# jinbeizame007/pytorch-r2d2-DPG

Hardware: NVIDIA H100
Metric: learner sequence-steps/sec (batch x seq_len) (higher is better)
Workload: dtype bf16x3 (fp32 operands split into bf16 hi+lo, three tensor-core passes, fp32 accumulate: ~16-bit operands)

## Files before the change

### pytorch-r2d2-dpg_b200/csrc/lstm_scan.cu

```cuda
#include <cooperative_groups.h>
#include <stdlib.h>

#include "gemm.cuh"
#include "lstm_scan.cuh"
#include "elementwise.cuh"
#include "sm90.cuh"

namespace cg = cooperative_groups;

namespace r2d2 {
namespace {

constexpr int SCAN_THREADS = 256;
constexpr int UNITS_PER_CTA = 32;
constexpr int ROWS_PER_CTA = 128;
constexpr int GT_LD = ROWS_PER_CTA + 4;
constexpr int DG_LD = ROWS_PER_CTA + 8;
constexpr unsigned long long kWaitLimitNs = 4000000000ull;

__device__ unsigned g_scan_status = 0;

__device__ __forceinline__ float accurate_sigmoid(float x) { return 1.0f / (1.0f + expf(-x)); }

__device__ __forceinline__ unsigned long long global_ns() {
  unsigned long long t;
  asm volatile("mov.u64 %0, %globaltimer;" : "=l"(t));
  return t;
}

__device__ __forceinline__ void wait_slice(uint64_t* bar, uint32_t parity) {
  if (sm90::mbar_try_wait(bar, parity)) return;
  if (*reinterpret_cast<volatile unsigned*>(&g_scan_status)) return;
  const unsigned long long t0 = global_ns();
  while (!sm90::mbar_try_wait(bar, parity)) {
    if (global_ns() - t0 > kWaitLimitNs) {
      atomicExch(&g_scan_status, 1u);
      return;
    }
  }
}

__device__ __forceinline__ uint32_t slice_parity(int s) { return (uint32_t)((s - 1) >> 1) & 1u; }

template <int H> __host__ __device__ constexpr bool w_hi_in_smem() { return H > 256; }

template <int H, int NB>
struct FwdSmem {
  static constexpr int C = H / 32;
  static constexpr int HROW = UNITS_PER_CTA + 8;
  static constexpr int SLICE = 2 * NB * HROW;
  static constexpr int W_BYTES = w_hi_in_smem<H>() ? (H / 16) * 8 * 32 * 16 : 0;
  static constexpr int HB_ELEMS = 2 * C * SLICE;
  static constexpr int GT_ELEMS = NB * GT_LD;
  static constexpr int HS_ELEMS = SLICE;
  static constexpr int BAR_OFF = W_BYTES + HB_ELEMS * 2 + GT_ELEMS * 4 + HS_ELEMS * 2;
  static constexpr int BYTES = BAR_OFF + 2 * C * 8;
  static_assert((SLICE * 2) % 16 == 0 && BAR_OFF % 16 == 0, "bulk copies need 16-byte granules");
  static_assert(BYTES <= 232448, "forward scan tile does not fit in 227 KB of shared memory");
};

template <int H, int NB>
__global__ void __launch_bounds__(SCAN_THREADS, 1) lstm_scan_fwd_kernel(ScanFwdParams p) {
  constexpr int C = H / 32, KS = H / 16, NT = NB / 8;
  constexpr bool WS = w_hi_in_smem<H>();
  using SM = FwdSmem<H, NB>;
  constexpr int HROW = SM::HROW, SLICE = SM::SLICE;
  cg::cluster_group cluster = cg::this_cluster();
  const int rank = (int)cluster.block_rank();
  const int b0 = (blockIdx.x / C) * NB;
  const int tid = threadIdx.x, lane = tid & 31, w = tid >> 5;
  const int g = lane >> 2, c = lane & 3;
  const int B = p.B, S = p.T * p.repeat;

  extern __shared__ __align__(16) unsigned char smem_raw[];
  uint4* w_hi_s = reinterpret_cast<uint4*>(smem_raw);
  __nv_bfloat16* hb = reinterpret_cast<__nv_bfloat16*>(smem_raw + SM::W_BYTES);
  float* gt = reinterpret_cast<float*>(smem_raw + SM::W_BYTES + SM::HB_ELEMS * 2);
  __nv_bfloat16* hstage = reinterpret_cast<__nv_bfloat16*>(smem_raw + SM::W_BYTES + SM::HB_ELEMS * 2 + SM::GT_ELEMS * 4);
  uint64_t* bar = reinterpret_cast<uint64_t*>(smem_raw + SM::BAR_OFF);

  for (int idx = tid; idx < NB * H; idx += SCAN_THREADS) {
    const int n = idx / H, k = idx % H, b = b0 + n;
    float v = (b < B && p.h0) ? __ldg(p.h0 + (size_t)b * H + k) : 0.f;
    __nv_bfloat16 hi, lo;
    split_bf16(v, hi, lo);
    __nv_bfloat16* row = hb + (0 * C + k / UNITS_PER_CTA) * SLICE + n * HROW + k % UNITS_PER_CTA;
    row[0] = hi;
    row[NB * HROW] = lo;
  }
  const int ug = rank * 32 + lane;
  float cst[NT];
#pragma unroll
  for (int e = 0; e < NT; ++e) {
    const int b = b0 + w + 8 * e;
    cst[e] = 0.f;
    if (b < B) {
      float hv = p.h0 ? __ldg(p.h0 + (size_t)b * H + ug) : 0.f;
      float cv = p.c0 ? __ldg(p.c0 + (size_t)b * H + ug) : 0.f;
      p.hs[(size_t)b * H + ug] = hv;
      p.cs[(size_t)b * H + ug] = cv;
      cst[e] = cv;
    }
  }
  if (tid < 2 * C) {
    sm90::mbar_init(bar + tid, 1);
    sm90::fence_mbar_init_cluster();
    sm90::mbar_arrive_expect_tx(bar + tid, SLICE * 2);
  }

  uint32_t a_hi[WS ? 1 : KS][4], a_lo[KS][4];
  {
    const int gate = w >> 1;
    const int u_lo = (w & 1) * 16 + g;
    const float* w_r0 = p.whh + (size_t)(gate * H + rank * 32 + u_lo) * H;
    const float* w_r1 = w_r0 + (size_t)8 * H;
#pragma unroll
    for (int ks = 0; ks < KS; ++ks) {
      const int k = ks * 16 + 2 * c;
      float2 v0 = __ldg(reinterpret_cast<const float2*>(w_r0 + k));
      float2 v1 = __ldg(reinterpret_cast<const float2*>(w_r1 + k));
      float2 v2 = __ldg(reinterpret_cast<const float2*>(w_r0 + k + 8));
      float2 v3 = __ldg(reinterpret_cast<const float2*>(w_r1 + k + 8));
      uint32_t h[4];
      split_pack2(v0.x, v0.y, h[0], a_lo[ks][0]);
      split_pack2(v1.x, v1.y, h[1], a_lo[ks][1]);
      split_pack2(v2.x, v2.y, h[2], a_lo[ks][2]);
      split_pack2(v3.x, v3.y, h[3], a_lo[ks][3]);
      if constexpr (WS) {
        w_hi_s[(ks * 8 + w) * 32 + lane] = make_uint4(h[0], h[1], h[2], h[3]);
      } else {
#pragma unroll
        for (int f = 0; f < 4; ++f) a_hi[ks][f] = h[f];
      }
    }
  }
  __syncthreads();
  cluster.sync();

  const size_t gstride = (size_t)4 * H;
  for (int s = 0; s < S; ++s) {
    const int cur = s & 1, nxt = cur ^ 1;
    const int t = s / p.repeat;

#pragma unroll
    for (int nt = 0; nt < NT; ++nt)
#pragma unroll
      for (int f = 0; f < 4; ++f) {
        const int n = nt * 8 + 2 * c + (f & 1), r = 16 * w + g + (f >> 1) * 8, b = b0 + n;
        if (b < B) sm90::cp_async_4(gt + n * GT_LD + r, p.gin + ((size_t)t * B + b) * gstride + (r >> 5) * H + rank * 32 + (r & 31));
      }
    sm90::cp_async_commit();

    float acc[NT][4];
#pragma unroll
    for (int nt = 0; nt < NT; ++nt)
#pragma unroll
      for (int e = 0; e < 4; ++e) acc[nt][e] = 0.f;
    const __nv_bfloat16* hb_cur = hb + cur * C * SLICE;
    uint64_t* bar_cur = bar + cur * C;
    const uint32_t parity = slice_parity(s);
#pragma unroll
    for (int ks = 0; ks < KS; ++ks) {
      if ((ks & 1) == 0 && s > 0) wait_slice(bar_cur + ks / 2, parity);
      const __nv_bfloat16* hb_hi = hb_cur + (ks / 2) * SLICE;
      const __nv_bfloat16* hb_lo = hb_hi + NB * HROW;
      uint32_t ah[4];
      if constexpr (WS) {
        const uint4 v = w_hi_s[(ks * 8 + w) * 32 + lane];
        ah[0] = v.x; ah[1] = v.y; ah[2] = v.z; ah[3] = v.w;
      } else {
#pragma unroll
        for (int f = 0; f < 4; ++f) ah[f] = a_hi[ks][f];
      }
#pragma unroll
      for (int nt = 0; nt < NT; ++nt) {
        const int off = (nt * 8 + g) * HROW + (ks & 1) * 16 + 2 * c;
        uint32_t bh[2], bl[2];
        bh[0] = *reinterpret_cast<const uint32_t*>(hb_hi + off);
        bh[1] = *reinterpret_cast<const uint32_t*>(hb_hi + off + 8);
        bl[0] = *reinterpret_cast<const uint32_t*>(hb_lo + off);
        bl[1] = *reinterpret_cast<const uint32_t*>(hb_lo + off + 8);
        mma_bf16_16816(acc[nt], a_lo[ks], bh);
        mma_bf16_16816(acc[nt], ah, bl);
        mma_bf16_16816(acc[nt], ah, bh);
      }
    }
    sm90::cp_async_wait_all();
#pragma unroll
    for (int nt = 0; nt < NT; ++nt) {
      const int n = nt * 8 + 2 * c, r = 16 * w + g;
      gt[n * GT_LD + r] += acc[nt][0];
      gt[(n + 1) * GT_LD + r] += acc[nt][1];
      gt[n * GT_LD + r + 8] += acc[nt][2];
      gt[(n + 1) * GT_LD + r + 8] += acc[nt][3];
    }
    if (w == 0 && lane < C) sm90::bulk_wait_read_all();
    __syncthreads();
    if (s > 0 && tid < C) sm90::mbar_arrive_expect_tx(bar_cur + tid, SLICE * 2);

#pragma unroll
    for (int e = 0; e < NT; ++e) {
      const int n = w + 8 * e, b = b0 + n;
      __nv_bfloat16 hi = __float2bfloat16_rn(0.f), lo = hi;
      if (b < B) {
        const float* gr = gt + n * GT_LD + lane;
        const float ig = accurate_sigmoid(gr[0]);
        const float fg = accurate_sigmoid(gr[32]);
        const float gg = tanhf(gr[64]);
        const float og = accurate_sigmoid(gr[96]);
        const float cn = fg * cst[e] + ig * gg;
        const float hn = og * tanhf(cn);
        cst[e] = cn;
        if (!p.no_save) {
          float* go = p.gates + ((size_t)s * B + b) * gstride + ug;
          go[0] = ig; go[H] = fg; go[2 * H] = gg; go[3 * H] = og;
          p.cs[((size_t)(s + 1) * B + b) * H + ug] = cn;
        }
        p.hs[((size_t)(s + 1) * B + b) * H + ug] = hn;
        if (p.head_in && (s % p.repeat) == p.repeat - 1)
          p.head_in[((size_t)t * B + b) * H + ug] = tanhf(hn);
        split_bf16(hn, hi, lo);
      }
      hstage[(0 * NB + n) * HROW + lane] = hi;
      hstage[(1 * NB + n) * HROW + lane] = lo;
    }
    sm90::fence_proxy_async_smem();
    __syncthreads();

    if (s + 1 < S && w == 0 && lane < C) {
      const uint32_t slot = sm90::smem_u32(hb + (nxt * C + rank) * SLICE);
      const uint32_t slot_bar = sm90::smem_u32(bar + nxt * C + rank);
      sm90::bulk_copy_s2cluster(sm90::map_cluster(slot, lane), sm90::smem_u32(hstage), SLICE * 2,
                                sm90::map_cluster(slot_bar, lane));
      sm90::bulk_commit();
    }
  }
  cluster.sync();
}

template <int H, int NB>
struct BwdSmem {
  static constexpr int C = H / 32;
  static constexpr int DG_ELEMS = 2 * NB * DG_LD;
  static constexpr int PS_LD = NB + 2;
  static constexpr int PS_ELEMS = 2 * C * UNITS_PER_CTA * PS_LD;
  static constexpr int PS_BYTES_PER_SRC = UNITS_PER_CTA * NB * 4;
  static constexpr int MT = (H / 16 + 7) / 8;
  static constexpr int W_BYTES = w_hi_in_smem<H>() ? MT * 8 * 8 * 32 * 16 : 0;
  static constexpr int BAR_OFF = W_BYTES + DG_ELEMS * 2 + PS_ELEMS * 4;
  static constexpr int BYTES = BAR_OFF + 2 * C * 8;
  static_assert(BAR_OFF % 8 == 0, "mbarrier alignment");
  static_assert(BYTES <= 232448, "BPTT scan tile does not fit in 227 KB of shared memory");
};

template <int H, int NB>
__global__ void __launch_bounds__(SCAN_THREADS, 1) lstm_scan_bwd_kernel(ScanBwdParams p) {
  constexpr int C = H / 32, NT = NB / 8;
  constexpr int M_TILES = H / 16;
  constexpr int MT = (M_TILES + 7) / 8;
  constexpr int KS = ROWS_PER_CTA / 16;
  constexpr bool WS = w_hi_in_smem<H>();
  using SM = BwdSmem<H, NB>;
  cg::cluster_group cluster = cg::this_cluster();
  const int rank = (int)cluster.block_rank();
  const int b0 = (blockIdx.x / C) * NB;
  const int tid = threadIdx.x, lane = tid & 31, w = tid >> 5;
  const int g = lane >> 2, c = lane & 3;
  const int B = p.B, S = p.T * p.repeat;

  extern __shared__ __align__(16) unsigned char smem_raw[];
  uint4* w_hi_s = reinterpret_cast<uint4*>(smem_raw);
  __nv_bfloat16* dgs = reinterpret_cast<__nv_bfloat16*>(smem_raw + SM::W_BYTES);
  float* ps = reinterpret_cast<float*>(smem_raw + SM::W_BYTES + SM::DG_ELEMS * 2);
  uint64_t* bar = reinterpret_cast<uint64_t*>(smem_raw + SM::BAR_OFF);

  if (tid < 2 * C) {
    sm90::mbar_init(bar + tid, 1);
    sm90::fence_mbar_init_cluster();
    sm90::mbar_arrive_expect_tx(bar + tid, SM::PS_BYTES_PER_SRC);
  }

  uint32_t a_hi[WS ? 1 : MT][WS ? 1 : KS][4], a_lo[MT][KS][4];
#pragma unroll
  for (int i = 0; i < MT; ++i) {
    const int mi = w * MT + i;
#pragma unroll
    for (int ks = 0; ks < KS; ++ks) {
      uint32_t h[4];
#pragma unroll
      for (int f = 0; f < 4; ++f) {
        float v0 = 0.f, v1 = 0.f;
        if (mi < M_TILES) {
          const int j = mi * 16 + g + (f & 1) * 8;
          const int r = ks * 16 + 2 * c + (f >> 1) * 8;
          const size_t row0 = (size_t)((r >> 5) * H + rank * 32 + (r & 31));
          v0 = __ldg(p.whh + row0 * H + j);
          v1 = __ldg(p.whh + (row0 + 1) * H + j);
        }
        split_pack2(v0, v1, h[f], a_lo[i][ks][f]);
      }
      if constexpr (WS) {
        w_hi_s[((i * KS + ks) * 8 + w) * 32 + lane] = make_uint4(h[0], h[1], h[2], h[3]);
      } else {
#pragma unroll
        for (int f = 0; f < 4; ++f) a_hi[i][ks][f] = h[f];
      }
    }
  }

  __syncthreads();
  const int ug = rank * 32 + lane;
  const size_t gstride = (size_t)4 * H;
  float dcn[NT], keep[NT][4];
#pragma unroll
  for (int e = 0; e < NT; ++e) {
    dcn[e] = 0.f;
#pragma unroll
    for (int q = 0; q < 4; ++q) keep[e][q] = 0.f;
  }
  cluster.sync();

  for (int it = 0; it < S; ++it) {
    const int s = S - 1 - it;
    const int buf = it & 1;
    const int t = s / p.repeat;
    const int rel = s - p.head_first_step;
    const bool has_head = p.dh_head && rel >= 0 && (rel % p.repeat) == p.repeat - 1;

    if (it > 0) {
      const uint32_t parity = slice_parity(it);
#pragma unroll
      for (int src = 0; src < C; ++src) wait_slice(bar + buf * C + src, parity);
    }

#pragma unroll
    for (int e = 0; e < NT; ++e) {
      const int n = w + 8 * e, b = b0 + n;
      float dg[4] = {0.f, 0.f, 0.f, 0.f};
      if (b < B) {
        float dh = 0.f;
        if (it > 0) {
#pragma unroll
          for (int src = 0; src < C; ++src) dh += ps[((buf * C + src) * UNITS_PER_CTA + lane) * SM::PS_LD + n];
        }
        if (has_head) dh += __ldg(p.dh_head + ((size_t)(rel / p.repeat) * B + b) * H + ug);
        const float* gs = p.gates + ((size_t)s * B + b) * gstride + ug;
        const float ig = gs[0], fg = gs[H], gg = gs[2 * H], og = gs[3 * H];
        const float c_prev = __ldg(p.cs + ((size_t)s * B + b) * H + ug);
        const float tc = tanhf(__ldg(p.cs + ((size_t)(s + 1) * B + b) * H + ug));
        const float dc = dcn[e] + dh * og * (1.f - tc * tc);
        dg[3] = dh * tc * og * (1.f - og);
        dg[0] = dc * gg * ig * (1.f - ig);
        dg[1] = dc * c_prev * fg * (1.f - fg);
        dg[2] = dc * ig * (1.f - gg * gg);
        dcn[e] = dc * fg;
        float* go = p.dgates + ((size_t)s * B + b) * gstride + ug;
        go[0] = dg[0]; go[H] = dg[1]; go[2 * H] = dg[2]; go[3 * H] = dg[3];
        if (p.repeat > 1) {
#pragma unroll
          for (int q = 0; q < 4; ++q) keep[e][q] += dg[q];
          if (s % p.repeat == 0) {
            float* gi = p.dgin + ((size_t)t * B + b) * gstride + ug;
#pragma unroll
            for (int q = 0; q < 4; ++q) { gi[q * H] = keep[e][q]; keep[e][q] = 0.f; }
          }
        }
      }
#pragma unroll
      for (int q = 0; q < 4; ++q) {
        __nv_bfloat16 hi, lo;
        split_bf16(dg[q], hi, lo);
        dgs[(0 * NB + n) * DG_LD + q * 32 + lane] = hi;
        dgs[(1 * NB + n) * DG_LD + q * 32 + lane] = lo;
      }
    }
    __syncthreads();
    if (it > 0 && tid < C) sm90::mbar_arrive_expect_tx(bar + buf * C + tid, SM::PS_BYTES_PER_SRC);

    if (s > 0) {
      float acc[MT][NT][4];
#pragma unroll
      for (int i = 0; i < MT; ++i)
#pragma unroll
        for (int nt = 0; nt < NT; ++nt)
#pragma unroll
          for (int e = 0; e < 4; ++e) acc[i][nt][e] = 0.f;
      const __nv_bfloat16* d_hi = dgs;
      const __nv_bfloat16* d_lo = dgs + NB * DG_LD;
#pragma unroll
      for (int ks = 0; ks < KS; ++ks) {
        uint32_t bh[NT][2], bl[NT][2];
#pragma unroll
        for (int nt = 0; nt < NT; ++nt) {
          const int off = (nt * 8 + g) * DG_LD + ks * 16 + 2 * c;
          bh[nt][0] = *reinterpret_cast<const uint32_t*>(d_hi + off);
          bh[nt][1] = *reinterpret_cast<const uint32_t*>(d_hi + off + 8);
          bl[nt][0] = *reinterpret_cast<const uint32_t*>(d_lo + off);
          bl[nt][1] = *reinterpret_cast<const uint32_t*>(d_lo + off + 8);
        }
#pragma unroll
        for (int i = 0; i < MT; ++i) {
          uint32_t ah[4];
          if constexpr (WS) {
            const uint4 v = w_hi_s[((i * KS + ks) * 8 + w) * 32 + lane];
            ah[0] = v.x; ah[1] = v.y; ah[2] = v.z; ah[3] = v.w;
          } else {
#pragma unroll
            for (int f = 0; f < 4; ++f) ah[f] = a_hi[i][ks][f];
          }
#pragma unroll
          for (int nt = 0; nt < NT; ++nt) {
            mma_bf16_16816(acc[i][nt], a_lo[i][ks], bh[nt]);
            mma_bf16_16816(acc[i][nt], ah, bl[nt]);
            mma_bf16_16816(acc[i][nt], ah, bh[nt]);
          }
        }
      }
      const uint32_t slot_bar = sm90::smem_u32(bar + (buf ^ 1) * C + rank);
#pragma unroll
      for (int i = 0; i < MT; ++i) {
        const int mi = w * MT + i;
        if (mi < M_TILES) {
#pragma unroll
          for (int h2 = 0; h2 < 2; ++h2) {
            const int j = mi * 16 + g + h2 * 8;
            const int owner = j >> 5, jl = j & 31;
            const uint32_t slot = sm90::map_cluster(
                sm90::smem_u32(ps + (((buf ^ 1) * C + rank) * UNITS_PER_CTA + jl) * SM::PS_LD), owner);
            const uint32_t owner_bar = sm90::map_cluster(slot_bar, owner);
#pragma unroll
            for (int nt = 0; nt < NT; ++nt)
              sm90::st_async_f2(slot + (nt * 8 + 2 * c) * 4, acc[i][nt][2 * h2], acc[i][nt][2 * h2 + 1], owner_bar);
          }
        }
      }
    }
    __syncthreads();
  }
  cluster.sync();
}

__global__ void lstm_cell_fwd_pointwise(const float* __restrict__ gpre, const float* __restrict__ c_prev,
                                        float* __restrict__ gates, float* __restrict__ h_out,
                                        float* __restrict__ c_out, float* __restrict__ head_in, int B, int H) {
  const int idx = blockIdx.x * blockDim.x + threadIdx.x;
  if (idx >= B * H) return;
  const int b = idx / H, u = idx % H;
  const float* gr = gpre + (size_t)b * 4 * H + u;
  const float ig = accurate_sigmoid(gr[0]), fg = accurate_sigmoid(gr[H]);
  const float gg = tanhf(gr[2 * H]), og = accurate_sigmoid(gr[3 * H]);
  const float cn = fg * c_prev[idx] + ig * gg;
  const float hn = og * tanhf(cn);
  float* go = gates + (size_t)b * 4 * H + u;
  go[0] = ig; go[H] = fg; go[2 * H] = gg; go[3 * H] = og;
  h_out[idx] = hn;
  c_out[idx] = cn;
  if (head_in) head_in[idx] = tanhf(hn);
}

__global__ void lstm_cell_bwd_pointwise(const float* __restrict__ gates, const float* __restrict__ c_prev,
                                        const float* __restrict__ c_new, const float* __restrict__ dh_head,
                                        const float* __restrict__ dh_rec, float* __restrict__ dc_state,
                                        float* __restrict__ dgates, float* __restrict__ dgin, int dgin_mode,
                                        int B, int H) {
  const int idx = blockIdx.x * blockDim.x + threadIdx.x;
  if (idx >= B * H) return;
  const int b = idx / H, u = idx % H;
  const float* gs = gates + (size_t)b * 4 * H + u;
  const float ig = gs[0], fg = gs[H], gg = gs[2 * H], og = gs[3 * H];
  float dh = dh_rec ? dh_rec[idx] : 0.f;
  if (dh_head) dh += dh_head[idx];
  const float tc = tanhf(c_new[idx]);
  const float dc = dc_state[idx] + dh * og * (1.f - tc * tc);
  float dg[4];
  dg[3] = dh * tc * og * (1.f - og);
  dg[0] = dc * gg * ig * (1.f - ig);
  dg[1] = dc * c_prev[idx] * fg * (1.f - fg);
  dg[2] = dc * ig * (1.f - gg * gg);
  dc_state[idx] = dc * fg;
  float* go = dgates + (size_t)b * 4 * H + u;
  float* gi = dgin ? dgin + (size_t)b * 4 * H + u : nullptr;
#pragma unroll
  for (int q = 0; q < 4; ++q) {
    go[q * H] = dg[q];
    if (dgin_mode == 1) gi[q * H] = dg[q];
    else if (dgin_mode == 2) gi[q * H] += dg[q];
  }
}

int scan_forward_generic(const ScanFwdParams& p, float* scratch, cudaStream_t stream) {
  const int B = p.B, H = p.H, S = p.T * p.repeat;
  const size_t bh = (size_t)B * H;
  R2D2_REQUIRE(scratch != nullptr, "generic scan needs scratch");
  if (p.h0) R2D2_CUDA_TRY(cudaMemcpyAsync(p.hs, p.h0, bh * 4, cudaMemcpyDeviceToDevice, stream));
  else R2D2_CUDA_TRY(cudaMemsetAsync(p.hs, 0, bh * 4, stream));
  if (p.c0) R2D2_CUDA_TRY(cudaMemcpyAsync(p.cs, p.c0, bh * 4, cudaMemcpyDeviceToDevice, stream));
  else R2D2_CUDA_TRY(cudaMemsetAsync(p.cs, 0, bh * 4, stream));
  const int blocks = ceil_div((int)bh, 256);
  for (int s = 0; s < S; ++s) {
    const int t = s / p.repeat;
    GemmParams g;
    g.A = p.hs + (size_t)s * bh; g.lda = H;
    g.B = p.whh; g.ldb = H;
    g.C = scratch; g.ldc = 4 * H;
    g.M = B; g.N = 4 * H; g.K = H;
    g.Z = p.gin + (size_t)t * B * 4 * H; g.ldz = 4 * H;
    g.epilogue = EPI_ADD_Z;
    R2D2_TRY(gemm_f32(g, GEMM_NT, stream));
    float* head = (p.head_in && (s % p.repeat) == p.repeat - 1) ? p.head_in + (size_t)t * bh : nullptr;
    lstm_cell_fwd_pointwise<<<blocks, 256, 0, stream>>>(scratch, p.cs + (size_t)s * bh,
                                                         p.gates + (size_t)s * B * 4 * H, p.hs + (size_t)(s + 1) * bh,
                                                         p.cs + (size_t)(s + 1) * bh, head, B, H);
    count_launch();
  }
  R2D2_CUDA_TRY(cudaGetLastError());
  return R2D2_OK;
}

int scan_backward_generic(const ScanBwdParams& p, cudaStream_t stream) {
  const int B = p.B, H = p.H, S = p.T * p.repeat;
  const size_t bh = (size_t)B * H;
  R2D2_REQUIRE(p.scratch != nullptr, "generic scan needs scratch");
  float* dh_rec = p.scratch;
  float* dc_state = p.scratch + bh;
  R2D2_CUDA_TRY(cudaMemsetAsync(p.scratch, 0, 2 * bh * 4, stream));
  const int blocks = ceil_div((int)bh, 256);
  for (int s = S - 1; s >= 0; --s) {
    const int t = s / p.repeat;
    const int rel = s - p.head_first_step;
    const bool has_head = p.dh_head && rel >= 0 && (rel % p.repeat) == p.repeat - 1;
    const float* head = has_head ? p.dh_head + (size_t)(rel / p.repeat) * bh : nullptr;
    int mode = 0;
    if (p.repeat > 1) mode = ((s % p.repeat) == p.repeat - 1) ? 1 : 2;
    lstm_cell_bwd_pointwise<<<blocks, 256, 0, stream>>>(
        p.gates + (size_t)s * B * 4 * H, p.cs + (size_t)s * bh, p.cs + (size_t)(s + 1) * bh, head,
        (s == S - 1) ? nullptr : dh_rec, dc_state, p.dgates + (size_t)s * B * 4 * H,
        mode ? p.dgin + (size_t)t * B * 4 * H : nullptr, mode, B, H);
    count_launch();
    if (s > 0) {
      GemmParams g;
      g.A = p.dgates + (size_t)s * B * 4 * H; g.lda = 4 * H;
      g.B = p.whh; g.ldb = H;
      g.C = dh_rec; g.ldc = H;
      g.M = B; g.N = H; g.K = 4 * H;
      R2D2_TRY(gemm_f32(g, GEMM_NN, stream));
    }
  }
  R2D2_CUDA_TRY(cudaGetLastError());
  return R2D2_OK;
}

template <typename Kern>
int set_cluster_attributes(Kern kern, int cluster_size, int smem_bytes) {
  R2D2_CUDA_TRY(cudaFuncSetAttribute(kern, cudaFuncAttributeMaxDynamicSharedMemorySize, smem_bytes));
  if (cluster_size > 8) R2D2_CUDA_TRY(cudaFuncSetAttribute(kern, cudaFuncAttributeNonPortableClusterSizeAllowed, 1));
  return R2D2_OK;
}

cudaLaunchConfig_t cluster_config(int cluster_size, int n_clusters, int smem_bytes, cudaStream_t stream,
                                  cudaLaunchAttribute* attr) {
  cudaLaunchConfig_t cfg = {};
  cfg.gridDim = dim3(cluster_size * n_clusters);
  cfg.blockDim = dim3(SCAN_THREADS);
  cfg.dynamicSmemBytes = smem_bytes;
  cfg.stream = stream;
  attr[0].id = cudaLaunchAttributeClusterDimension;
  attr[0].val.clusterDim.x = cluster_size;
  attr[0].val.clusterDim.y = 1;
  attr[0].val.clusterDim.z = 1;
  cfg.attrs = attr;
  cfg.numAttrs = 1;
  return cfg;
}

template <typename Kern, typename Params>
int launch_cluster(Kern kern, const Params& p, int cluster_size, int n_clusters, int smem_bytes, cudaStream_t stream) {
  R2D2_TRY(set_cluster_attributes(kern, cluster_size, smem_bytes));
  cudaLaunchAttribute attr[1];
  cudaLaunchConfig_t cfg = cluster_config(cluster_size, n_clusters, smem_bytes, stream, attr);
  R2D2_CUDA_TRY(cudaLaunchKernelEx(&cfg, kern, p));
  count_launch();
  return R2D2_OK;
}

template <typename Kern>
int resident_clusters(Kern kern, int cluster_size, int smem_bytes, int* out) {
  R2D2_TRY(set_cluster_attributes(kern, cluster_size, smem_bytes));
  cudaLaunchAttribute attr[1];
  cudaLaunchConfig_t cfg = cluster_config(cluster_size, 1, smem_bytes, nullptr, attr);
  R2D2_CUDA_TRY(cudaOccupancyMaxActiveClusters(out, kern, &cfg));
  return R2D2_OK;
}

template <int H, typename K8, typename K16, typename K32>
int pick_nb(int B, K8 k8, int smem8, K16 k16, int smem16, K32 k32, int smem32, int* nb) {
  int fit = 0;
  R2D2_TRY(resident_clusters(k8, H / 32, smem8, &fit));
  if (ceil_div(B, 8) <= fit) { *nb = 8; return R2D2_OK; }
  R2D2_TRY(resident_clusters(k16, H / 32, smem16, &fit));
  if (ceil_div(B, 16) <= fit || !k32) { *nb = 16; return R2D2_OK; }
  *nb = 32;
  (void)smem32;
  return R2D2_OK;
}

template <int H>
int fwd_dispatch(const ScanFwdParams& p, cudaStream_t stream) {
  constexpr bool WIDE = !w_hi_in_smem<H>();
  constexpr int NB3 = WIDE ? 32 : 16;
  int nb = 0;
  R2D2_TRY(pick_nb<H>(p.B, lstm_scan_fwd_kernel<H, 8>, FwdSmem<H, 8>::BYTES, lstm_scan_fwd_kernel<H, 16>,
                      FwdSmem<H, 16>::BYTES, WIDE ? lstm_scan_fwd_kernel<H, NB3> : nullptr, FwdSmem<H, NB3>::BYTES, &nb));
  if (nb == 8)
    return launch_cluster(lstm_scan_fwd_kernel<H, 8>, p, H / 32, ceil_div(p.B, 8), FwdSmem<H, 8>::BYTES, stream);
  if (nb == 16)
    return launch_cluster(lstm_scan_fwd_kernel<H, 16>, p, H / 32, ceil_div(p.B, 16), FwdSmem<H, 16>::BYTES, stream);
  return launch_cluster(lstm_scan_fwd_kernel<H, NB3>, p, H / 32, ceil_div(p.B, NB3), FwdSmem<H, NB3>::BYTES, stream);
}
template <int H>
int bwd_dispatch(const ScanBwdParams& p, cudaStream_t stream) {
  constexpr bool WIDE = !w_hi_in_smem<H>();
  constexpr int NB3 = WIDE ? 32 : 16;
  int nb = 0;
  R2D2_TRY(pick_nb<H>(p.B, lstm_scan_bwd_kernel<H, 8>, BwdSmem<H, 8>::BYTES, lstm_scan_bwd_kernel<H, 16>,
                      BwdSmem<H, 16>::BYTES, WIDE ? lstm_scan_bwd_kernel<H, NB3> : nullptr, BwdSmem<H, NB3>::BYTES, &nb));
  if (nb == 8)
    return launch_cluster(lstm_scan_bwd_kernel<H, 8>, p, H / 32, ceil_div(p.B, 8), BwdSmem<H, 8>::BYTES, stream);
  if (nb == 16)
    return launch_cluster(lstm_scan_bwd_kernel<H, 16>, p, H / 32, ceil_div(p.B, 16), BwdSmem<H, 16>::BYTES, stream);
  return launch_cluster(lstm_scan_bwd_kernel<H, NB3>, p, H / 32, ceil_div(p.B, NB3), BwdSmem<H, NB3>::BYTES, stream);
}

}

bool lstm_scan_cluster_supported(int H) { return H == 32 || H == 64 || H == 128 || H == 256 || H == 512; }

static int g_scan_impl = -1;
void lstm_scan_set_impl(int impl) { g_scan_impl = impl ? 1 : 0; }
int lstm_scan_get_impl() {
  if (g_scan_impl < 0) {
    const char* e = getenv("R2D2_SCAN_IMPL");
    g_scan_impl = (e && (e[0] == 's' || e[0] == '0')) ? 0 : 1;
  }
  return g_scan_impl;
}
static bool use_cluster_kernels(int H) { return lstm_scan_cluster_supported(H) && lstm_scan_get_impl() == 1; }

int lstm_scan_error_status(int* out, cudaStream_t stream) {
  R2D2_REQUIRE(out, "null");
  unsigned v = 0;
  R2D2_CUDA_TRY(cudaMemcpyFromSymbolAsync(&v, g_scan_status, sizeof(v), 0, cudaMemcpyDeviceToHost, stream));
  R2D2_CUDA_TRY(cudaStreamSynchronize(stream));
  *out = (int)v;
  return R2D2_OK;
}

size_t lstm_scan_fwd_scratch_floats(int B, int H) { return (size_t)B * 4 * H; }
size_t lstm_scan_bwd_scratch_floats(int B, int H) { return (size_t)2 * B * H; }

int lstm_scan_forward(const ScanFwdParams& p, cudaStream_t stream) {
  R2D2_REQUIRE(p.gin && p.whh && p.gates && p.hs && p.cs, "null pointer");
  R2D2_REQUIRE(p.T > 0 && p.B > 0 && p.H > 0 && p.repeat >= 1, "shape");
  R2D2_REQUIRE(p.repeat == 1 || p.gates != p.gin, "gates must not alias gin when repeat > 1");
  if (use_cluster_kernels(p.H)) {
    switch (p.H) {
      case 32: return fwd_dispatch<32>(p, stream);
      case 64: return fwd_dispatch<64>(p, stream);
      case 128: return fwd_dispatch<128>(p, stream);
      case 256: return fwd_dispatch<256>(p, stream);
      case 512: return fwd_dispatch<512>(p, stream);
      default: break;
    }
  }
  return scan_forward_generic(p, p.scratch, stream);
}

int lstm_scan_backward(const ScanBwdParams& p, cudaStream_t stream) {
  R2D2_REQUIRE(p.gates && p.hs && p.cs && p.whh && p.dgates, "null pointer");
  R2D2_REQUIRE(p.T > 0 && p.B > 0 && p.H > 0 && p.repeat >= 1, "shape");
  R2D2_REQUIRE(p.repeat == 1 || (p.dgin && p.dgin != p.dgates), "dgin buffer required when repeat > 1");
  int rc = R2D2_OK;
  switch (use_cluster_kernels(p.H) ? p.H : 0) {
    case 32: rc = bwd_dispatch<32>(p, stream); break;
    case 64: rc = bwd_dispatch<64>(p, stream); break;
    case 128: rc = bwd_dispatch<128>(p, stream); break;
    case 256: rc = bwd_dispatch<256>(p, stream); break;
    case 512: rc = bwd_dispatch<512>(p, stream); break;
    default: rc = scan_backward_generic(p, stream); break;
  }
  R2D2_TRY(rc);
  if (p.dbias) {
    const float* src = p.repeat > 1 ? p.dgin : p.dgates;
    R2D2_TRY(colsum(src, 4 * p.H, p.T * p.B, 4 * p.H, p.dbias, p.dbias2, stream));
  }
  return R2D2_OK;
}

}
```

Baseline: 1.009 million.

## Prefetch next step's gates and cell states into shared memory via cp.async in BPTT scan

The backward LSTM scan now issues cp.async loads of the next timestep's gates, previous cell state and head gradient into a shared-memory staging buffer before the recurrent GEMM, then reads them from smem after waiting. This overlaps the global-memory latency on the serial critical path with tensor-core work. It also carries c_new in registers instead of reloading cs[s+1] each step, and simplifies the weight-load address math. The extra staging buffer increases shared-memory use, and since only one stage is staged, the buffer must not be overwritten while it is still being read.

```diff
diff --git a/pytorch-r2d2-dpg_b200/csrc/lstm_scan.cu b/pytorch-r2d2-dpg_b200/csrc/lstm_scan.cu
--- a/pytorch-r2d2-dpg_b200/csrc/lstm_scan.cu
+++ b/pytorch-r2d2-dpg_b200/csrc/lstm_scan.cu
@@ -247,7 +247,9 @@
   static constexpr int PS_BYTES_PER_SRC = UNITS_PER_CTA * NB * 4;
   static constexpr int MT = (H / 16 + 7) / 8;
   static constexpr int W_BYTES = w_hi_in_smem<H>() ? MT * 8 * 8 * 32 * 16 : 0;
-  static constexpr int BAR_OFF = W_BYTES + DG_ELEMS * 2 + PS_ELEMS * 4;
+  static constexpr int STAGE_PLANES = 6;
+  static constexpr int STAGE_ELEMS = STAGE_PLANES * NB * UNITS_PER_CTA;
+  static constexpr int BAR_OFF = W_BYTES + DG_ELEMS * 2 + PS_ELEMS * 4 + STAGE_ELEMS * 4;
   static constexpr int BYTES = BAR_OFF + 2 * C * 8;
   static_assert(BAR_OFF % 8 == 0, "mbarrier alignment");
   static_assert(BYTES <= 232448, "BPTT scan tile does not fit in 227 KB of shared memory");
@@ -272,14 +274,44 @@
   uint4* w_hi_s = reinterpret_cast<uint4*>(smem_raw);
   __nv_bfloat16* dgs = reinterpret_cast<__nv_bfloat16*>(smem_raw + SM::W_BYTES);
   float* ps = reinterpret_cast<float*>(smem_raw + SM::W_BYTES + SM::DG_ELEMS * 2);
+  float* stage = ps + SM::PS_ELEMS;
   uint64_t* bar = reinterpret_cast<uint64_t*>(smem_raw + SM::BAR_OFF);
+  constexpr int PLANE = NB * UNITS_PER_CTA;
+  constexpr size_t gstride = (size_t)4 * H;
+
+  auto head_step = [&](int s) {
+    const int rel = s - p.head_first_step;
+    return p.dh_head && rel >= 0 && (rel % p.repeat) == p.repeat - 1;
+  };
+  auto prefetch = [&](int s) {
+    const int rel = s - p.head_first_step;
+    const bool head = head_step(s);
+    unsigned tv;
+    asm volatile("mov.u32 %0, %%tid.x;" : "=r"(tv));
+    const int lane = tv & 31, w = tv >> 5, ug = rank * 32 + lane;
+#pragma unroll
+    for (int e = 0; e < NT; ++e) {
+      const int n = w + 8 * e, b = b0 + n;
+      if (b < B) {
+        float* st = stage + n * UNITS_PER_CTA + lane;
+        const float* gs = p.gates + ((size_t)s * B + b) * gstride + ug;
+#pragma unroll
+        for (int q = 0; q < 4; ++q) sm90::cp_async_4(st + q * PLANE, gs + q * H);
+        sm90::cp_async_4(st + 4 * PLANE, p.cs + ((size_t)s * B + b) * H + ug);
+        if (head) sm90::cp_async_4(st + 5 * PLANE, p.dh_head + ((size_t)(rel / p.repeat) * B + b) * H + ug);
+      }
+    }
+    sm90::cp_async_commit();
+  };
 
   if (tid < 2 * C) {
     sm90::mbar_init(bar + tid, 1);
     sm90::fence_mbar_init_cluster();
     sm90::mbar_arrive_expect_tx(bar + tid, SM::PS_BYTES_PER_SRC);
   }
-
+  prefetch(S - 1);
+
+  const float* w_t = p.whh + (size_t)(rank * 32 + 2 * c) * H + w * MT * 16 + g;
   uint32_t a_hi[WS ? 1 : MT][WS ? 1 : KS][4], a_lo[MT][KS][4];
 #pragma unroll
   for (int i = 0; i < MT; ++i) {
@@ -291,11 +323,9 @@
       for (int f = 0; f < 4; ++f) {
         float v0 = 0.f, v1 = 0.f;
         if (mi < M_TILES) {
-          const int j = mi * 16 + g + (f & 1) * 8;
-          const int r = ks * 16 + 2 * c + (f >> 1) * 8;
-          const size_t row0 = (size_t)((r >> 5) * H + rank * 32 + (r & 31));
-          v0 = __ldg(p.whh + row0 * H + j);
-          v1 = __ldg(p.whh + (row0 + 1) * H + j);
+          const float* w0 = w_t + ((ks >> 1) * H + (ks & 1) * 16 + (f >> 1) * 8) * H + i * 16 + (f & 1) * 8;
+          v0 = __ldg(w0);
+          v1 = __ldg(w0 + H);
         }
         split_pack2(v0, v1, h[f], a_lo[i][ks][f]);
       }
@@ -310,11 +340,12 @@
 
   __syncthreads();
   const int ug = rank * 32 + lane;
-  const size_t gstride = (size_t)4 * H;
-  float dcn[NT], keep[NT][4];
+  float dcn[NT], keep[NT][4], c_new[NT];
 #pragma unroll
   for (int e = 0; e < NT; ++e) {
+    const int b = b0 + w + 8 * e;
     dcn[e] = 0.f;
+    c_new[e] = b < B ? __ldg(p.cs + ((size_t)S * B + b) * H + ug) : 0.f;
 #pragma unroll
     for (int q = 0; q < 4; ++q) keep[e][q] = 0.f;
   }
@@ -324,30 +355,35 @@
     const int s = S - 1 - it;
     const int buf = it & 1;
     const int t = s / p.repeat;
-    const int rel = s - p.head_first_step;
-    const bool has_head = p.dh_head && rel >= 0 && (rel % p.repeat) == p.repeat - 1;
-
+    const bool has_head = head_step(s);
+
+    float dh_rec[NT];
+#pragma unroll
+    for (int e = 0; e < NT; ++e) dh_rec[e] = 0.f;
     if (it > 0) {
       const uint32_t parity = slice_parity(it);
 #pragma unroll
-      for (int src = 0; src < C; ++src) wait_slice(bar + buf * C + src, parity);
-    }
+      for (int src = 0; src < C; ++src) {
+        wait_slice(bar + buf * C + src, parity);
+        const float* pr = ps + ((buf * C + src) * UNITS_PER_CTA + lane) * SM::PS_LD + w;
+#pragma unroll
+        for (int e = 0; e < NT; ++e) dh_rec[e] += pr[8 * e];
+      }
+    }
+    sm90::cp_async_wait_all();
 
 #pragma unroll
     for (int e = 0; e < NT; ++e) {
       const int n = w + 8 * e, b = b0 + n;
       float dg[4] = {0.f, 0.f, 0.f, 0.f};
       if (b < B) {
-        float dh = 0.f;
-        if (it > 0) {
-#pragma unroll
-          for (int src = 0; src < C; ++src) dh += ps[((buf * C + src) * UNITS_PER_CTA + lane) * SM::PS_LD + n];
-        }
-        if (has_head) dh += __ldg(p.dh_head + ((size_t)(rel / p.repeat) * B + b) * H + ug);
-        const float* gs = p.gates + ((size_t)s * B + b) * gstride + ug;
-        const float ig = gs[0], fg = gs[H], gg = gs[2 * H], og = gs[3 * H];
-        const float c_prev = __ldg(p.cs + ((size_t)s * B + b) * H + ug);
-        const float tc = tanhf(__ldg(p.cs + ((size_t)(s + 1) * B + b) * H + ug));
+        const float* st = stage + n * UNITS_PER_CTA + lane;
+        float dh = dh_rec[e];
+        if (has_head) dh += st[5 * PLANE];
+        const float ig = st[0], fg = st[PLANE], gg = st[2 * PLANE], og = st[3 * PLANE];
+        const float c_prev = st[4 * PLANE];
+        const float tc = tanhf(c_new[e]);
+        c_new[e] = c_prev;
         const float dc = dcn[e] + dh * og * (1.f - tc * tc);
         dg[3] = dh * tc * og * (1.f - og);
         dg[0] = dc * gg * ig * (1.f - ig);
@@ -378,6 +414,7 @@
     if (it > 0 && tid < C) sm90::mbar_arrive_expect_tx(bar + buf * C + tid, SM::PS_BYTES_PER_SRC);
 
     if (s > 0) {
+      prefetch(s - 1);
       float acc[MT][NT][4];
 #pragma unroll
       for (int i = 0; i < MT; ++i)
```

Result: faster. 1.053 million (median of 6 runs) (+4.4%).
